# danini/pose-graph-initialization

Measured on AMD Instinct MI355X. Metric: pose-graph edges/sec (essential+decompose), higher is better.
Workload: dtype f32 scoring / f64 solver; 1 GPU; configs[1]: 10000 pairs x 2000 corrs batched essential RANSAC + decompose per GPU; pairs_per_gpu=10000, corrs_per_pair=2000, mode=adaptive (confidence 0.99, cap 1000, rounds of 32), parallelism=pairs sharded over 1 GPU(s), exchange=none (single GPU)

## Files before the change

pose-graph-initialization_amd/csrc/pgi_kernels.hip:

```cpp
#include "pgi_device.hpp"
#include "pgi_internal.hpp"

#include <algorithm>
#include <condition_variable>
#include <mutex>
#include <new>
#include <string>
#include <thread>
#include <vector>
#include <cstdio>
#include <cstdlib>
#include <cstring>

namespace pgi {

constexpr int kMaxNW = 4;
constexpr uint32_t kNw1Pairs = 98304, kNw2Pairs = 12288;
constexpr int QCAP = 40;
constexpr double QMAGIC = 393216.0;

struct GcCtx {
    uint32_t* prev;
    uint32_t* msg;
    uint8_t* lab;
    uint32_t* last;
    const float* e_lds;
    uint32_t lambda64;
    uint32_t built;
};

template <int NW>
struct WgShared {
    float bestE[9];
    int best_score;
    uint32_t best_ninl;
    float candE[NW][9];
    int cand_score[NW];
    uint32_t cand_ninl[NW];
    uint32_t cand_hyp[NW];
    uint32_t wave_cnt[NW];
    uint32_t votes[4];
    uint32_t q_count[NW];
    uint32_t q_hyp[NW][QCAP];
    uint32_t pass_ctr;
    uint32_t nbar;
    uint32_t mask_cnt;
    int lo_score;
    uint32_t lo_ninl, lo_ni, lo_runs;
    float loE[9];
    double Rt[21];
    GcCtx gc;
};

struct K1Args {
    const float* x1;
    const float* y1;
    const float* x2;
    const float* y2;
    const uint64_t* off;
    const double* thr;
    const double* guess;
    const uint8_t* has_guess;
    pgi_edge* edges;
    uint8_t* masks;
    uint32_t n_pairs;
    uint32_t pts_cap;
    uint64_t pair_id_base;
    uint64_t seed;
    pgi_params prm;
    unsigned long long* prof;
    const uint32_t* pair_list;
    const uint32_t* pair_count;
    uint32_t* pair_head;
    const float* src_x1;
    const float* src_y1;
    const float* src_x2;
    const float* src_y2;
    uint32_t* gc_prev;
    uint32_t* gc_msg;
    uint32_t gc_lds_off;
};

template <int LDS_PTS>
struct Rows {
    const float4* lds;
    const float* x1;
    const float* y1;
    const float* x2;
    const float* y2;
    uint32_t n;
    uint32_t lds_n;
    PGI_DEV float4 get(uint32_t i) const {
        if constexpr (LDS_PTS == 1) {
            return lds[i];
        } else if constexpr (LDS_PTS == 2) {
            if (i < lds_n) return lds[i];
            const float nanv = __builtin_nanf("");
            if (i < n) return make_float4(x1[i], y1[i], x2[i], y2[i]);
            return make_float4(nanv, nanv, nanv, nanv);
        } else {
            const float nanv = __builtin_nanf("");
            if (i < n) return make_float4(x1[i], y1[i], x2[i], y2[i]);
            return make_float4(nanv, nanv, nanv, nanv);
// ... 187 lines not shown
        base -= 64u;
        const uint32_t i = base + (uint32_t)lane;
        const bool valid = i < n;
        const uint32_t w = valid ? gc_load(g.msg + i) : 0u;
        const uint32_t pv = valid ? gc_load(g.prev + i) : kGcNone;
        const uint32_t k = gc_word_k(w) & 31u;
        const int d = gc_word_delta(w);
        succ_of[lane] = 64u;
        wave_sync();
        if (valid && pv != kGcNone && pv >= base) succ_of[pv - base] = (uint32_t)lane;
        wave_sync();
        const uint32_t succ = succ_of[lane];
        wave_sync();
        uint32_t lab = (w >> 6) & 1u;
        if (succ == 64u && !((w >> 5) & 1u)) lab = d < 0 ? 1u : 0u;
        bool done = !valid || succ == 64u;
        const int sl = succ == 64u ? 0 : (int)succ;
        for (;;) {
            const uint64_t dm = __ballot(done);
            if (dm == ~0ull) break;
            const uint32_t ls = (uint32_t)__shfl((int)lab, sl), ks = (uint32_t)__shfl((int)k, sl);
            if (!done && ((dm >> sl) & 1ull)) {
                lab = gc_prev_label(ls, ks, d, k, lam);
                done = true;
            }
        }
        if (valid && pv != kGcNone && pv < base) {
            const uint32_t wp = gc_load(g.msg + pv);
            gc_store(g.msg + pv, wp | 32u | (gc_prev_label(lab, k, gc_word_delta(wp), gc_word_k(wp) & 31u, lam) << 6));
        }
        if (valid) g.lab[i] = (uint8_t)lab;
        cnt += (uint32_t)__popcll(__ballot(valid && lab));
        asm volatile("s_waitcnt vmcnt(0)" ::: "memory");
    }
    wave_sync();
    return cnt;
}

template <int LDS_PTS>
__device__ __noinline__ uint32_t gc_label_rows(const float4* lds, const float* x1, const float* y1, const float* x2, const float* y2, uint32_t n,
                                               uint32_t lds_n, uint32_t npad, float thr2, GcCtx* gp, int lane) {
    Rows<LDS_PTS> rows;
    rows.lds = lds;
    rows.x1 = x1; rows.y1 = y1; rows.x2 = x2; rows.y2 = y2;
    rows.n = n;
    rows.lds_n = lds_n;
    return gc_label_wave<LDS_PTS>(&rows, n, npad, thr2, gp, lane);
}

template <int LDS_PTS>
PGI_DEV uint32_t normal_matrix_wave(const Rows<LDS_PTS>& rows, uint32_t npad, const float E[9], float tau2,
                                    double* loA, double* tri, int lane, const uint8_t* lab = nullptr) {
    uint32_t cnt = 0;
#pragma unroll
    for (int blk = 0; blk < 3; ++blk) {
        constexpr int kLo[3] = {0, 17, 35}, kRow0[3] = {0, 2, 5}, kRow1[3] = {2, 5, 9}, kCnt[3] = {17, 18, 10};
        double S[18];
#pragma unroll
        for (int i = 0; i < 18; ++i) S[i] = 0.0;
        for (uint32_t base = 0; base < npad; base += 64) {
            const float4 p = rows.get(base + lane);
            float r2, den;
            sampson_terms(E, p.x, p.y, p.z, p.w, r2, den);
            const bool in = lab ? (base + (uint32_t)lane < rows.n && lab[base + lane] != 0) : (r2 < tau2 * den);
            if (blk == 0) cnt += __popcll(__ballot(in));
            if (in) {
                const double x1 = p.x, y1 = p.y, x2 = p.z, y2 = p.w;
                double a[9];
                a[0] = x2 * x1; a[1] = x2 * y1; a[2] = x2;
                a[3] = y2 * x1; a[4] = y2 * y1; a[5] = y2;
                a[6] = x1;      a[7] = y1;      a[8] = 1.0;
                constexpr int kTri[9] = {0, 9, 17, 24, 30, 35, 39, 42, 44};
#pragma unroll
                for (int ii = kRow0[blk]; ii < kRow1[blk]; ++ii)
#pragma unroll
                    for (int jj = ii; jj < 9; ++jj) {
                        const int k = kTri[ii] + (jj - ii) - kLo[blk];
                        double t = a[ii] * a[jj];
                        t = (t + QMAGIC) - QMAGIC;
                        S[k] = S[k] + t;
                    }
            }
        }
#pragma unroll
        for (int i = 0; i < kCnt[blk]; ++i) {
            const double v = wave_sum_exact(S[i]);
            if (lane == 0) tri[kLo[blk] + i] = v;
        }
    }
    wave_sync();
    if (lane < 45) {
        int i = 0, rem = lane;
        while (rem >= 9 - i) {
            rem -= 9 - i;
            ++i;
        }
        const int j = i + rem;
        const double v = tri[lane];
        loA[9 * i + j] = v;
        loA[9 * j + i] = v;
    }
    wave_sync();
    return cnt;
}

template <int LDS_PTS, int NW>
PGI_DEV uint32_t normal_matrix_wg(const Rows<LDS_PTS>& rows, uint32_t npad, const float E[9], float tau2,
                                  double* loA, double* partial, WgShared<NW>* sh, int tid) {
    constexpr int NT = NW * 64;
    const int lane = tid & 63, w = tid >> 6;
    uint32_t cnt = 0;
#pragma unroll
    for (int blk = 0; blk < 3; ++blk) {
        constexpr int kLo[3] = {0, 17, 35}, kRow0[3] = {0, 2, 5}, kRow1[3] = {2, 5, 9}, kCnt[3] = {17, 18, 10};
        double S[18];
#pragma unroll
        for (int i = 0; i < 18; ++i) S[i] = 0.0;
        for (uint32_t base = 0; base < npad; base += NT) {
            const uint32_t i = base + tid;
            const float nanv = __builtin_nanf("");
            const float4 p = (i < npad) ? rows.get(i) : make_float4(nanv, nanv, nanv, nanv);
            float r2, den;
            sampson_terms(E, p.x, p.y, p.z, p.w, r2, den);
            const bool in = r2 < tau2 * den;
            if (blk == 0) cnt += __popcll(__ballot(in));
            if (in) {
                const double x1 = p.x, y1 = p.y, x2 = p.z, y2 = p.w;
                double a[9];
                a[0] = x2 * x1; a[1] = x2 * y1; a[2] = x2;
                a[3] = y2 * x1; a[4] = y2 * y1; a[5] = y2;
                a[6] = x1;      a[7] = y1;      a[8] = 1.0;
                constexpr int kTri[9] = {0, 9, 17, 24, 30, 35, 39, 42, 44};
#pragma unroll
                for (int ii = kRow0[blk]; ii < kRow1[blk]; ++ii)
#pragma unroll
                    for (int jj = ii; jj < 9; ++jj) {
                        const int k = kTri[ii] + (jj - ii) - kLo[blk];
                        double t = a[ii] * a[jj];
                        t = (t + QMAGIC) - QMAGIC;
                        S[k] = S[k] + t;
                    }
            }
        }
#pragma unroll
        for (int i = 0; i < kCnt[blk]; ++i) {
            const double v = wave_sum_exact(S[i]);
            if (lane == 0) partial[45 * w + kLo[blk] + i] = v;
        }
    }
    if (lane == 0) sh->wave_cnt[w] = cnt;
    __syncthreads();
    if (tid < 45) {
        double v = partial[tid];
#pragma unroll
        for (int ww = 1; ww < NW; ++ww) v = v + partial[45 * ww + tid];
        int i = 0, rem = tid;
        while (rem >= 9 - i) {
            rem -= 9 - i;
            ++i;
        }
        const int j = i + rem;
        loA[9 * i + j] = v;
        loA[9 * j + i] = v;
    }
    uint32_t total = 0;
#pragma unroll
    for (int ww = 0; ww < NW; ++ww) total += sh->wave_cnt[ww];
    __syncthreads();
    return total;
}

PGI_DEV void jacobi9_wave(double* A, double* V, double* basis0, int lane) {
    for (int i = lane; i < 81; i += 64) V[i] = (i % 10 == 0) ? 1.0 : 0.0;
    wave_sync();
    const int m = lane / 9, l = lane - 9 * m;
    const bool act = lane < 36;
    int pr = act ? m + 1 : 1, qr = act ? 8 - m : 8;
    for (int sw = 0; sw < kJacobiSweeps; ++sw)
        for (int r = 0; r < 9; ++r) {
            const int p = min(pr, qr), q = max(pr, qr);
            pr = pr == 8 ? 0 : pr + 1;
            qr = qr == 8 ? 0 : qr + 1;
            double c = 1.0, s = 0.0;
            if (act) {
                const double apq = A[9 * p + q];
                if (apq != 0.0) {
                    const double al = A[10 * q] - A[10 * p], be = 2.0 * apq;
                    const double h = sqrt(fma(al, al, be * be));
                    const double d = fabs(al) + h;
                    const double r = sqrt(fma(d, d, be * be));
                    const double inv = 1.0 / r;
                    c = d * inv;
                    s = (al >= 0.0 ? be : -be) * inv;
                }
            }
            wave_sync();
            if (act) {
                const double ap = A[9 * l + p], aq = A[9 * l + q];
                A[9 * l + p] = fma(c, ap, -(s * aq));
                A[9 * l + q] = fma(s, ap, c * aq);
                const double vp = V[9 * l + p], vq = V[9 * l + q];
                V[9 * l + p] = fma(c, vp, -(s * vq));
                V[9 * l + q] = fma(s, vp, c * vq);
            }
            wave_sync();
            if (act) {
                const double ap = A[9 * p + l], aq = A[9 * q + l];
                A[9 * p + l] = fma(c, ap, -(s * aq));
                A[9 * q + l] = fma(s, ap, c * aq);
            }
            wave_sync();
        }
    double d[9];
#pragma unroll
    for (int i = 0; i < 9; ++i) d[i] = A[10 * i];
    uint32_t taken = 0;
// ... 90 lines not shown
    double* wscr = wscr_all + w * W_DOUBLES;
    float* queue = reinterpret_cast<float*>(wscr + W_REGA);

    Rows<LDS_PTS> rows;
    rows.lds = pts;
    rows.x1 = a.x1 + o; rows.y1 = a.y1 + o; rows.x2 = a.x2 + o; rows.y2 = a.y2 + o;
    rows.n = n;
    rows.lds_n = LDS_PTS != 0 ? min(npad, a.pts_cap) : 0u;

    pgi_edge* edge = a.edges + pair;
    uint8_t* mask = a.masks + o;
    Prof prof;
    prof.start();

    if (LDS_PTS == 1 && npad > a.pts_cap) {
        for (uint32_t i = tid; i < n; i += NT) mask[i] = 0;
        if (tid == 0) {
            edge_clear(edge);
            edge->status = PGI_EDGE_TOO_MANY_ROWS;
        }
        return;
    }
    {
        const bool direct = a.src_x1 != nullptr;
        const float* sx1 = direct ? a.src_x1 + o : rows.x1;
        const float* sy1 = direct ? a.src_y1 + o : rows.y1;
        const float* sx2 = direct ? a.src_x2 + o : rows.x2;
        const float* sy2 = direct ? a.src_y2 + o : rows.y2;
        if constexpr (LDS_PTS != 0) {
            const float nanv = __builtin_nanf("");
            for (uint32_t i = tid; i < rows.lds_n; i += NT)
                pts[i] = (i < n) ? make_float4(sx1[i], sy1[i], sx2[i], sy2[i]) : make_float4(nanv, nanv, nanv, nanv);
        }
        if constexpr (LDS_PTS != 1) {
            if (direct) {
                float* mx1 = const_cast<float*>(rows.x1);
                float* my1 = const_cast<float*>(rows.y1);
                float* mx2 = const_cast<float*>(rows.x2);
                float* my2 = const_cast<float*>(rows.y2);
                for (uint32_t i = rows.lds_n + tid; i < n; i += NT) {
                    mx1[i] = sx1[i];
                    my1[i] = sy1[i];
                    mx2[i] = sx2[i];
                    my2[i] = sy2[i];
                }
            }
        }
    }
    if (tid == 0) {
        sh->best_score = -1;
        sh->best_ninl = 0;
        sh->votes[0] = sh->votes[1] = sh->votes[2] = sh->votes[3] = 0;
        sh->mask_cnt = 0;
        sh->pass_ctr = 0;
        sh->nbar = 0;
        sh->lo_runs = 0;
        if (a.gc_prev) {
            sh->gc.prev = a.gc_prev + o;
            sh->gc.msg = a.gc_msg + o;
            sh->gc.lab = mask;
            sh->gc.last = reinterpret_cast<uint32_t*>(smem + a.gc_lds_off);
            sh->gc.e_lds = sh->bestE;
            sh->gc.lambda64 = min(a.prm.lo_graph_cut, 255u);
            sh->gc.built = 0;
        }
    }
    __syncthreads();
    prof.mark<0>();

    const double thr = a.thr[pair];
    const float thr2 = (float)(thr * thr);
    const pgi_params prm = a.prm;

    if (n < 5) {
        for (uint32_t i = tid; i < n; i += NT) mask[i] = 0;
        if (tid == 0) {
            edge_clear(edge);
            edge->status = PGI_EDGE_FEW_POINTS;
        }
        return;
    }

    uint32_t out_iters = 0, out_lo = 0, out_used_guess = 0, out_score = 0;
    float mask_tau2 = thr2;
    bool success = false, have_model = false;
    uint32_t guess_ninl = 0;

    bool guided_done = false;
    auto local_optimise = [&]() {
        if constexpr (!GUESS) return;
        int ni_first = -1;
        GcCtx* const gc = a.gc_prev ? &sh->gc : nullptr;
        if constexpr (NW > 1) {
            if (prm.lo_iters && !gc) {
                float bE0[9];
#pragma unroll
                for (int c = 0; c < 9; ++c) bE0[c] = sh->bestE[c];
                int td = tid;
                asm volatile("" : "+v"(td));
                ni_first = (int)normal_matrix_wg<LDS_PTS, NW>(rows, npad, bE0, thr2, wscr_all + W_REGA + G_REGA_SZ, wscr_all + W_DOUBLES, sh, td);
            }
        }
        if (w == 0) {
            for (uint32_t it = 0; it < prm.lo_iters; ++it) {
                float bE[9];
#pragma unroll
                for (int c = 0; c < 9; ++c) bE[c] = sh->bestE[c];
                const int cur_best = __builtin_amdgcn_readfirstlane(sh->best_score);
// ... 14 lines not shown
                if (ln < 9) sh->bestE[ln] = reinterpret_cast<const float*>(wscr_all + W_REGA)[9 * r_idx + ln];
                wave_sync();
            }
        }
    };
    if (GUESS && a.has_guess[pair] && prm.guess_mode == 1u) {
        const double* G = a.guess + 12 * (size_t)pair;
        const double R[9] = {G[0], G[1], G[2], G[3], G[4], G[5], G[6], G[7], G[8]};
        const uint64_t rng_g = mix64(a.seed ^ mix64(a.pair_id_base + pair));
        int ln = lane;
        asm volatile("" : "+v"(ln));
        constexpr int kPerWave = 32 / NW;
        const bool mine = ln < kPerWave;
        const uint32_t h = (uint32_t)(w * kPerWave + (mine ? ln : 0));
        const uint32_t i0 = draw_index(rng_g, 0x40000000u + h, 0u, n);
        uint32_t i1 = i0;
        for (uint32_t k = 1; k < 64u && i1 == i0; ++k) i1 = draw_index(rng_g, 0x40000000u + h, k, n);
        double nv[2][3];
#pragma unroll
        for (int q = 0; q < 2; ++q) {
            const float4 p = rows.get(q == 0 ? i0 : i1);
            const double X1[3] = {(double)p.x, (double)p.y, 1.0}, X2[3] = {(double)p.z, (double)p.w, 1.0};
            double av[3];
#pragma unroll
            for (int i = 0; i < 3; ++i) av[i] = fma(R[3 * i], X1[0], fma(R[3 * i + 1], X1[1], R[3 * i + 2]));
            cross3(X2, av, nv[q]);
        }
        double t[3];
        cross3(nv[0], nv[1], t);
        const double t2 = fma(t[0], t[0], fma(t[1], t[1], t[2] * t[2]));
        const double tx[9] = {0, -t[2], t[1], t[2], 0, -t[0], -t[1], t[0], 0};
        double Eg[9], n2 = 0.0;
#pragma unroll
        for (int i = 0; i < 3; ++i)
#pragma unroll
            for (int j = 0; j < 3; ++j) {
                double sacc = 0;
#pragma unroll
                for (int k = 0; k < 3; ++k) sacc += tx[3 * i + k] * R[3 * k + j];
                Eg[3 * i + j] = sacc;
            }
#pragma unroll
        for (int m = 0; m < 9; ++m) n2 = fma(Eg[m], Eg[m], n2);
        const double inv = 1.0 / sqrt(n2);
        float E32[9];
#pragma unroll
        for (int m = 0; m < 9; ++m) E32[m] = (float)(Eg[m] * inv);
        const bool valid = mine && (t2 > 1e-30) && (n2 > 0.0);
        const int cnt = enqueue_models(valid, E32, h, queue, sh->q_hyp[w], ln);
        wave_sync();
        int gb_score = -1, gb_idx = -1;
        uint32_t gb_ninl = 0, gb_hyp = 0;
        score_queue<LDS_PTS>(rows, n, npad, queue, sh->q_hyp[w], 0, cnt, thr2, ln, -1, 0u, gb_score, gb_ninl, gb_hyp, gb_idx);
        if (gb_idx >= 0 && ln < 9) sh->candE[w][ln] = queue[9 * gb_idx + ln];
        if (lane == 0) {
            sh->cand_score[w] = gb_score;
            sh->cand_ninl[w] = gb_ninl;
            sh->cand_hyp[w] = gb_hyp;
        }
        __syncthreads();
        int rb = -1, rbw = -1;
        uint32_t rbh = 0;
#pragma unroll
        for (int ww = 0; ww < NW; ++ww) {
            const int cs = sh->cand_score[ww];
            const uint32_t ch = sh->cand_hyp[ww];
            if (cs > rb || (cs == rb && cs >= 0 && ch < rbh)) {
                rb = cs;
                rbw = ww;
                rbh = ch;
            }
        }
        __syncthreads();
        if (rb >= 0) {
            if (tid == 0) {
                sh->best_score = rb;
                sh->best_ninl = sh->cand_ninl[rbw];
#pragma unroll
                for (int c = 0; c < 9; ++c) sh->bestE[c] = sh->candE[rbw][c];
            }
            __syncthreads();
            local_optimise();
            __syncthreads();
            if (sh->best_ninl >= prm.min_inliers) {
                guided_done = true;
                have_model = true;
                out_used_guess = 1;
                out_iters = 32;
                out_lo = sh->lo_runs;
                out_score = (uint32_t)sh->best_score;
            }
        }
        if (!guided_done) {
            __syncthreads();
            if (tid == 0) {
                sh->best_score = -1;
                sh->best_ninl = 0;
                sh->lo_runs = 0;
            }
            __syncthreads();
        }
    }

    if (GUESS && a.has_guess[pair] && prm.guess_mode != 1u) {
        const double* G = a.guess + 12 * (size_t)pair;
        const double R[9] = {G[0], G[1], G[2], G[3], G[4], G[5], G[6], G[7], G[8]};
        const double t[3] = {G[9], G[10], G[11]};
        const double tx[9] = {0, -t[2], t[1], t[2], 0, -t[0], -t[1], t[0], 0};
        double Eg[9], n2 = 0.0;
#pragma unroll
        for (int i = 0; i < 3; ++i)
#pragma unroll
            for (int j = 0; j < 3; ++j) {
                double s = 0;
#pragma unroll
                for (int k = 0; k < 3; ++k) s += tx[3 * i + k] * R[3 * k + j];
                Eg[3 * i + j] = s;
            }
#pragma unroll
        for (int m = 0; m < 9; ++m) n2 = fma(Eg[m], Eg[m], n2);
        const double inv = 1.0 / sqrt(n2);
        float Ef[9];
#pragma unroll
        for (int m = 0; m < 9; ++m) Ef[m] = (float)(Eg[m] * inv);
        const double trunc = 1.5 * thr;
        const float tau2 = prm.guess_quirk ? (float)trunc : (float)(trunc * trunc);
        if (w == 0) {
            __builtin_amdgcn_s_setprio(3);
            int rs0, ri0;
            uint32_t rn0;
            const uint32_t ni0 = refit_wave0<LDS_PTS>(rows, n, npad, Ef, tau2, thr2, wscr_all, sh->q_hyp[0], lane, -1, 0u, rs0, rn0, ri0, prof);
            if (lane == 0) {
                sh->lo_ni = ni0;
                sh->lo_score = rs0;
                sh->lo_ninl = rn0;
            }
            if (ri0 >= 0 && lane < 9) sh->loE[lane] = reinterpret_cast<const float*>(wscr_all + W_REGA)[9 * ri0 + lane];
            __builtin_amdgcn_s_setprio(0);
        }
        __syncthreads();
        const uint32_t ni = sh->lo_ni;
        const int r_score = sh->lo_score;
        if (ni >= 5 && r_score >= 0 && ni >= prm.min_inliers) {
            success = true;
            have_model = true;
            out_used_guess = 1;
            out_lo = 1;
            out_score = (uint32_t)r_score;
            guess_ninl = ni;
            mask_tau2 = tau2;
            if (tid == 0) {
#pragma unroll
                for (int c = 0; c < 9; ++c) sh->bestE[c] = Ef[c];
            }
            __syncthreads();
        }
    }

    if (!success && !guided_done) {
        const uint64_t rng_base = mix64(a.seed ^ mix64(a.pair_id_base + pair));
        const uint32_t rs = prm.round_size ? prm.round_size : 32u;
        const uint32_t budget = prm.fixed_budget ? prm.fixed_budget : prm.max_iters;
        uint32_t hyps = 0;
        const uint32_t n_pass = (rs + 3u) / 4u;
        int wb_score = -1;
        uint32_t wb_ninl = 0, wb_hyp = 0;
        auto do_pass = [&](uint32_t pass, uint32_t base_hyp, int floor_score, uint32_t n_bar) {
            int ln = lane;
            asm volatile("" : "+v"(ln));
            const int g = ln >> 4, s = ln & 15;
            const uint32_t local = pass * 4 + g;
            const bool active = local < rs;
            const uint32_t hyp = base_hyp + (active ? local : 0u);
            const GroupScratch gs = group_scratch(wscr, g);
            uint32_t idx[5];
            sample5_group(rng_base, hyp, prm.sampler ? progressive_rows(hyp, n, prm.max_iters) : n, s, g * 16, ln,
                          reinterpret_cast<uint32_t*>(gs.rega), idx);
            uint32_t my = idx[0];
#pragma unroll
            for (int k = 1; k < 5; ++k)
                if (s == k) my = idx[k];
            const float4 mine = rows.get(my);
            prof.mark<1>();
            nullspace5_group(mine, s, g * 16, gs);
            prof.mark<2>();
            float E32[9];
            if constexpr (LDS_PTS != 1) {
                if (s < 5) smp_stash[(w * 4 + g) * 5 + s] = mine;
                wave_sync();
            }
            const bool valid = backend_group<false, 3, true>(
                gs, s, g * 16,
                [&](int i) {
                    if constexpr (LDS_PTS == 1) return rows.get(idx[i]);
                    else return smp_stash[(w * 4 + g) * 5 + i];
                },
                E32, nullptr, prof);
            wave_sync();
            const int cnt = enqueue_models(valid && active, E32, hyp, queue, sh->q_hyp[w], ln);
            wave_sync();
            prof.mark<9>();
            int bidx = -1;
            score_queue<LDS_PTS>(rows, n, npad, queue, sh->q_hyp[w], 0, cnt, thr2, ln, floor_score, n_bar, wb_score,
                                 wb_ninl, wb_hyp, bidx);
            if (bidx >= 0 && ln < 9) sh->candE[w][ln] = queue[9 * bidx + ln];
            wave_sync();
            prof.mark<10>();
        };
        auto pull_pass = [&]() -> uint32_t {
            uint32_t pass = 0;
            if (lane == 0) pass = atomicAdd(&sh->pass_ctr, 1u);
            return (uint32_t)__builtin_amdgcn_readfirstlane((int)pass);
        };
        int floor_score = -1;
        uint32_t n_bar = 0;
        bool deferred = false;
        auto terminated = [&](uint32_t at_hyps) {
            if (prm.fixed_budget || sh->best_score < 0 || sh->best_ninl < 5) return false;
            uint32_t nn = n;
            double conf = prm.confidence;
            asm volatile("" : "+s"(nn), "+s"(conf));
            const double rho = (double)sh->best_ninl / (double)nn;
            const double r5 = ((rho * rho) * (rho * rho)) * rho;
            const double q = 1.0 - r5;
            return pow_uint(q, at_hyps) <= 1.0 - conf;
        };
        while (hyps < budget) {
            for (;;) {
                const uint32_t pass = pull_pass();
                if (pass >= n_pass) break;
                do_pass(pass, hyps, floor_score, n_bar);
            }
            if (lane == 0) {
                sh->cand_score[w] = wb_score;
                sh->cand_ninl[w] = wb_ninl;
                sh->cand_hyp[w] = wb_hyp;
            }
            wb_score = -1;
            __syncthreads();
            prof.mark<22>();
            if (deferred) {
                deferred = false;
                if (terminated(hyps)) break;
            }
            hyps += rs;
            int rb = -1, rbw = -1;
            uint32_t rbh = 0;
#pragma unroll
            for (int ww = 0; ww < NW; ++ww) {
                const int cs = sh->cand_score[ww];
                const uint32_t ch = sh->cand_hyp[ww];
                if (cs > rb || (cs == rb && cs >= 0 && ch < rbh)) {
                    rb = cs;
                    rbw = ww;
                    rbh = ch;
                }
            }
            const bool improve = (rb >= 0) && (rb > sh->best_score);
            __syncthreads();
            if (tid == 0) {
                sh->pass_ctr = 0;
                if (improve) {
                    sh->best_score = rb;
                    sh->best_ninl = sh->cand_ninl[rbw];
                    sh->nbar = sh->cand_ninl[rbw];
#pragma unroll
                    for (int c = 0; c < 9; ++c) sh->bestE[c] = sh->candE[rbw][c];
                } else {
                    sh->nbar = sh->best_score >= 0 ? sh->best_ninl : 0u;
                }
            }
            __syncthreads();
            floor_score = __builtin_amdgcn_readfirstlane(sh->best_score);
            n_bar = (uint32_t)__builtin_amdgcn_readfirstlane((int)sh->nbar);
            if (improve) {
                int ni_first = -1;
                GcCtx* const gc = a.gc_prev ? &sh->gc : nullptr;
                if (NW > 1 && prm.lo_iters && !gc) {
                    float bE0[9];
#pragma unroll
                    for (int c = 0; c < 9; ++c) bE0[c] = sh->bestE[c];
                    const int td = (w << 6) + fresh_lane_id();
                    ni_first = (int)normal_matrix_wg<LDS_PTS, NW>(rows, npad, bE0, thr2, wscr_all + W_REGA + G_REGA_SZ,
                                                              wscr_all + W_DOUBLES, sh, td);
                }
                if (w == 0) {
                    __builtin_amdgcn_s_setprio(3);
                    for (uint32_t it = 0; it < prm.lo_iters; ++it) {
                        float bE[9];
#pragma unroll
                        for (int c = 0; c < 9; ++c) bE[c] = sh->bestE[c];
                        const int cur_best = __builtin_amdgcn_readfirstlane(sh->best_score);
                        const uint32_t cur_ninl = (uint32_t)__builtin_amdgcn_readfirstlane((int)sh->best_ninl);
                        int r_score, r_idx;
                        uint32_t r_ninl;
                        int ln = lane;
                        asm volatile("" : "+v"(ln));
                        const uint32_t ni = refit_wave0<LDS_PTS>(rows, n, npad, bE, thr2, thr2, wscr_all, sh->q_hyp[0], ln, cur_best,
                                                                       cur_ninl, r_score, r_ninl, r_idx, prof,
                                                                       it == 0 ? ni_first : -1, prm.lo_linear_pct, gc);
                        if (ni < 5) break;
                        if (lane == 0) sh->lo_runs += 1;
                        if (!(r_score > cur_best)) break;
                        if (lane == 0) {
                            sh->best_score = r_score;
                            sh->best_ninl = r_ninl;
                        }
                        if (ln < 9) sh->bestE[ln] = reinterpret_cast<const float*>(wscr_all + W_REGA)[9 * r_idx + ln];
                        wave_sync();
                    }
                    __builtin_amdgcn_s_setprio(0);
                }
                if constexpr (NW == 1) {
                    if (terminated(hyps)) break;
                } else {
                    deferred = true;
                }
            } else if (terminated(hyps)) {
                break;
            }
        }
        __syncthreads();
        out_lo = sh->lo_runs;
        out_iters = hyps;
        have_model = sh->best_score >= 0;
        if (have_model) out_score = (uint32_t)sh->best_score;
    }

    prof.mark<23>();
    const int ew = w, etid = (ew << 6) + fresh_lane_id(), elane = etid & 63;
    if (!have_model) {
        for (uint32_t i = etid; i < n; i += NT) mask[i] = 0;
        if (etid == 0) {
            edge_clear(edge);
            edge->status = PGI_EDGE_FEW_INLIERS;
            edge->iters = out_iters;
            edge->lo_runs = out_lo;
        }
        return;
    }
    const float* finalE = success ? sh->loE : sh->bestE;
    float maskE[9];
#pragma unroll
    for (int c = 0; c < 9; ++c) maskE[c] = sh->bestE[c];
    uint32_t mc = 0;
    if (ew == 0) decompose_wave(finalE, sh->Rt, elane);
    if (NW == 1 || ew != 0) {
        constexpr uint32_t kMaskLanes = NW == 1 ? 64u : (uint32_t)(NT - 64);
        for (uint32_t base = 0; base < npad; base += kMaskLanes) {
            const uint32_t i = base + (uint32_t)(NW == 1 ? etid : etid - 64);
            const float nanv = __builtin_nanf("");
            const float4 p = (i < npad) ? rows.get(i) : make_float4(nanv, nanv, nanv, nanv);
            float r2, den;
            sampson_terms(maskE, p.x, p.y, p.z, p.w, r2, den);
            const bool in = r2 < mask_tau2 * den;
            if (i < n) mask[i] = in ? 1 : 0;
            mc += __popcll(__ballot(in));
        }
        if (elane == 0) atomicAdd(&sh->mask_cnt, mc);
    }
    __syncthreads();
    double R1[9], R2[9], tt[3];
#pragma unroll
    for (int c = 0; c < 9; ++c) {
        R1[c] = sh->Rt[c];
        R2[c] = sh->Rt[9 + c];
    }
    tt[0] = sh->Rt[18]; tt[1] = sh->Rt[19]; tt[2] = sh->Rt[20];
    uint32_t v0 = 0, v1 = 0, v2 = 0, v3 = 0;
    for (uint32_t base = 0; base < npad; base += NT) {
        const uint32_t i = base + etid;
        const float nanv = __builtin_nanf("");
        const float4 p = (i < npad) ? rows.get(i) : make_float4(nanv, nanv, nanv, nanv);
        float r2, den;
        sampson_terms(maskE, p.x, p.y, p.z, p.w, r2, den);
        const bool in = r2 < mask_tau2 * den;
        const bool voter = (i < n) && (prm.vote_all_rows || in);
        uint32_t b1 = 0, b2 = 0;
        if (voter) {
            const double X1[3] = {p.x, p.y, 1.0}, X2[3] = {p.z, p.w, 1.0};
            double x2t[3];
            cross3(X2, tt, x2t);
            b1 = cheirality_bits(R1, tt, X1, X2, x2t);
            b2 = cheirality_bits(R2, tt, X1, X2, x2t);
        }
        v0 += __popcll(__ballot(b1 & 1u));
        v1 += __popcll(__ballot(b1 & 2u));
        v2 += __popcll(__ballot(b2 & 1u));
        v3 += __popcll(__ballot(b2 & 2u));
    }
    if (elane == 0) {
        atomicAdd(&sh->votes[0], v0);
        atomicAdd(&sh->votes[1], v1);
        atomicAdd(&sh->votes[2], v2);
        atomicAdd(&sh->votes[3], v3);
    }
    __syncthreads();
    if (etid == 0) {
        edge_clear(edge);
        const uint32_t n_inl = success ? guess_ninl : sh->mask_cnt;
#pragma unroll
        for (int c = 0; c < 9; ++c) edge->E[c] = (double)finalE[c];
        edge->n_inl = n_inl;
        edge->score = out_score;
        edge->iters = out_iters;
        edge->lo_runs = out_lo;
        edge->used_guess = out_used_guess;
        if (n_inl < prm.min_inliers) {
            edge->status = PGI_EDGE_FEW_INLIERS;
        } else {
            const uint32_t vt0 = sh->votes[0], vt1 = sh->votes[1], vt2 = sh->votes[2], vt3 = sh->votes[3];
            uint32_t best = 0, bv = vt0;
            if (vt1 > bv) { bv = vt1; best = 1; }
            if (vt2 > bv) { bv = vt2; best = 2; }
            if (vt3 > bv) { bv = vt3; best = 3; }
            const bool second = (best >> 1) != 0;
            bool bad = false;
#pragma unroll
            for (int c = 0; c < 9; ++c) {
                const double rv = second ? R2[c] : R1[c];
                edge->R[c] = rv;
                bad |= !(rv == rv);
            }
#pragma unroll
            for (int c = 0; c < 3; ++c) {
                edge->t[c] = (best & 1u) ? -tt[c] : tt[c];
                bad |= !(tt[c] == tt[c]);
            }
            edge->votes = bv;
            edge->cand = best;
// ... 1344 lines not shown
```

pose-graph-initialization_amd/csrc/pgi_device.hpp:

```cpp
#pragma once
#include <hip/hip_runtime.h>
#include <stdint.h>

#define PGI_DEV __device__ __forceinline__
#define PGI_PHASE __device__ __noinline__

namespace pgi {

constexpr int kGrid = 256;
constexpr int kNewton = 10;
constexpr int kJacobiSweeps = 6;
constexpr int kSvdSweeps = 4;
constexpr int kMaxModels = 10;

constexpr int kProfSlots = 32;
#ifdef PGI_PROFILE
struct Prof {
    unsigned long long t, acc[kProfSlots];
    PGI_DEV void start() {
        for (int i = 0; i < kProfSlots; ++i) acc[i] = 0;
        t = __builtin_amdgcn_s_memtime();
    }
    template <int I>
    PGI_DEV void mark() {
        const unsigned long long n = __builtin_amdgcn_s_memtime();
        acc[I] += n - t;
        t = n;
    }
    PGI_DEV void flush(unsigned long long* out, int lane) {
        if (out && lane == 0)
            for (int i = 0; i < kProfSlots; ++i) atomicAdd(out + i, acc[i]);
    }
};
#else
struct Prof {
    PGI_DEV void start() {}
    template <int I>
    PGI_DEV void mark() {}
    PGI_DEV void flush(unsigned long long*, int) {}
};
#endif

PGI_DEV void wave_sync() {
    __builtin_amdgcn_fence(__ATOMIC_RELEASE, "wavefront");
    __builtin_amdgcn_wave_barrier();
    __builtin_amdgcn_fence(__ATOMIC_ACQUIRE, "wavefront");
}

template <int CTRL>
PGI_DEV int dpp_i(int v) {
    return __builtin_amdgcn_update_dpp(0, v, CTRL, 0xF, 0xF, true);
}
template <int CTRL>
PGI_DEV double dpp_d(double v) {
    const int lo = __double2loint(v), hi = __double2hiint(v);
// ... 761 lines not shown
```

pose-graph-initialization_amd/pyposegraphbuilder/_lib.py:

```python
import ctypes as C
import os

import numpy as np

_PKG = os.path.dirname(os.path.abspath(__file__))
LIB_PATH = os.path.join(os.path.dirname(_PKG), "libpgi.so")
DBG_DOUBLES = 358


class Params(C.Structure):
    _fields_ = [("confidence", C.c_double), ("max_iters", C.c_uint32), ("round_size", C.c_uint32),
                ("lo_iters", C.c_uint32), ("min_inliers", C.c_uint32), ("fixed_budget", C.c_uint32),
                ("guess_quirk", C.c_uint32), ("vote_all_rows", C.c_uint32), ("guess_mode", C.c_uint32),
                ("lo_linear_pct", C.c_uint32), ("sampler", C.c_uint32), ("lo_graph_cut", C.c_uint32)]


class Edge(C.Structure):
    _fields_ = [("E", C.c_double * 9), ("R", C.c_double * 9), ("t", C.c_double * 3),
                ("status", C.c_int32), ("n_inl", C.c_uint32), ("score", C.c_uint32),
                ("iters", C.c_uint32), ("votes", C.c_uint32), ("cand", C.c_uint32),
                ("used_guess", C.c_uint32), ("lo_runs", C.c_uint32)]


class Batch(C.Structure):
# ... 182 lines not shown
    lib.pgi_five_point_batch.argtypes = [C.c_void_p, C.c_void_p, C.c_uint32, C.c_void_p, C.c_void_p, C.c_void_p]
    lib.pgi_rotation_average.argtypes = [C.c_void_p, C.c_void_p, C.c_uint32, C.c_uint32,
                                         C.POINTER(RotAvgParams), C.c_void_p, C.c_void_p]
    lib.pgi_default_rotavg_params.argtypes = [C.POINTER(RotAvgParams)]
    lib.pgi_default_transavg_params.argtypes = [C.POINTER(TransAvgParams)]
    lib.pgi_translation_average.argtypes = [C.c_void_p, C.c_void_p, C.c_uint32, C.c_uint32,
                                            C.POINTER(TransAvgParams), C.c_void_p, C.c_void_p]
    lib.pgi_translation_average_edges.argtypes = [C.c_void_p, C.c_void_p, C.c_void_p, C.c_void_p, C.c_void_p, C.c_uint32, C.c_uint32,
                                                  C.c_void_p, C.POINTER(TransAvgParams), C.c_void_p, C.c_void_p, C.c_void_p]
    lib.pgi_default_triangulate_params.restype = None
    lib.pgi_default_triangulate_params.argtypes = [C.POINTER(TriangulateParams)]
    view_args = [C.POINTER(KeypointView), C.c_void_p, C.c_void_p, C.c_void_p, C.c_uint32, C.POINTER(TriangulateParams)]
    lib.pgi_triangulate_tracks.argtypes = [C.c_void_p, C.c_void_p, C.c_void_p, C.c_uint32] + view_args + [C.c_void_p] * 6
    lib.pgi_tracklets_triangulate.argtypes = [C.c_void_p] + view_args + [C.c_void_p] * 6
    lib.pgi_default_bundle_params.restype = None
    lib.pgi_default_bundle_params.argtypes = [C.POINTER(BundleParams)]
    ba_args = [C.POINTER(KeypointView), C.c_void_p, C.c_void_p, C.c_void_p, C.c_void_p, C.c_uint32, C.POINTER(BundleParams),
               C.c_void_p, C.c_void_p, C.c_void_p, C.POINTER(BundleReport)]
    lib.pgi_bundle_adjust.argtypes = [C.c_void_p, C.c_void_p, C.c_void_p, C.c_uint32] + ba_args
    lib.pgi_tracklets_bundle_adjust.argtypes = [C.c_void_p] + ba_args
    baf_args = ba_args[:-1] + [C.c_void_p, C.c_void_p, C.c_uint32, C.POINTER(BundleReport), C.POINTER(C.c_uint32)]
    lib.pgi_bundle_adjust_focal.argtypes = [C.c_void_p, C.c_void_p, C.c_void_p, C.c_uint32] + baf_args
    lib.pgi_tracklets_bundle_adjust_focal.argtypes = [C.c_void_p] + baf_args
    lib.pgi_default_cycle_params.restype = None
    lib.pgi_default_cycle_params.argtypes = [C.POINTER(CycleParams)]
    lib.pgi_cycle_filter.argtypes = [C.c_void_p, C.c_void_p, C.c_uint32, C.c_uint32, C.POINTER(CycleParams), C.c_void_p, C.c_void_p,
                                     C.c_void_p, C.POINTER(CycleSummary)]
    lib.pgi_cycle_filter_edges.argtypes = [C.c_void_p, C.c_void_p, C.c_void_p, C.c_void_p, C.c_uint32, C.c_uint32, C.POINTER(CycleParams),
                                           C.c_void_p, C.c_void_p, C.c_void_p, C.POINTER(CycleSummary), C.c_void_p]
    _lib = lib
    return lib


def last_error():
    return load().pgi_last_error().decode()


def check(rc):
    if rc < 0:
        raise PgiError("pgi error %d: %s" % (rc, last_error()))
    return rc


def default_params(**kw):
    p = Params()
    load().pgi_default_params(C.byref(p))
    for k, v in kw.items():
        if not hasattr(p, k):
            raise TypeError("unknown parameter %r" % k)
        setattr(p, k, v)
    return p


def kernel_source_sha256(files=("csrc/pgi_kernels.hip", "csrc/pgi_device.hpp")):
    import hashlib
    h = hashlib.sha256()
    root = os.path.dirname(_PKG)
    for f in files:
        with open(os.path.join(root, f), "rb") as fh:
            h.update(fh.read())
    return h.hexdigest()
```

Baseline: 1.701 million edges/s.

## Double-buffer round candidates to drop a barrier and cache inlier bits

Candidate and pass-counter state is double-buffered by round parity. Each wave now reads the published best score and picks the round winner itself, which removes one of the two workgroup barriers per adaptive round. The normal-matrix builders keep the first block's inlier test as a per-lane bitmask and reuse it in later blocks instead of recomputing Sampson errors. The decompose vote pass reads inlier ballots stored in wave scratch during the mask pass, and the Rt buffer moves from shared state into scratch. This adds subtle cross-wave ordering assumptions and shrinks the shared struct, at the cost of more code complexity and possible race risk.

```diff
diff --git a/pose-graph-initialization_amd/csrc/pgi_kernels.hip b/pose-graph-initialization_amd/csrc/pgi_kernels.hip
--- a/pose-graph-initialization_amd/csrc/pgi_kernels.hip
+++ b/pose-graph-initialization_amd/csrc/pgi_kernels.hip
@@ -34,21 +34,21 @@
     float bestE[9];
     int best_score;
     uint32_t best_ninl;
-    float candE[NW][9];
-    int cand_score[NW];
-    uint32_t cand_ninl[NW];
-    uint32_t cand_hyp[NW];
+    float candE[2][NW][9];
+    int cand_score[2][NW];
+    uint32_t cand_ninl[2][NW];
+    uint32_t cand_hyp[2][NW];
+    int pub_score[2];
+    uint32_t pub_ninl[2];
     uint32_t wave_cnt[NW];
     uint32_t votes[4];
     uint32_t q_count[NW];
     uint32_t q_hyp[NW][QCAP];
-    uint32_t pass_ctr;
-    uint32_t nbar;
+    uint32_t pass_ctr[2];
     uint32_t mask_cnt;
     int lo_score;
     uint32_t lo_ninl, lo_ni, lo_runs;
     float loE[9];
-    double Rt[21];
     GcCtx gc;
 };
 
@@ -342,6 +342,7 @@
 PGI_DEV uint32_t normal_matrix_wave(const Rows<LDS_PTS>& rows, uint32_t npad, const float E[9], float tau2,
                                     double* loA, double* tri, int lane, const uint8_t* lab = nullptr) {
     uint32_t cnt = 0;
+    uint64_t inm = 0;
 #pragma unroll
     for (int blk = 0; blk < 3; ++blk) {
         constexpr int kLo[3] = {0, 17, 35}, kRow0[3] = {0, 2, 5}, kRow1[3] = {2, 5, 9}, kCnt[3] = {17, 18, 10};
@@ -350,9 +351,18 @@
         for (int i = 0; i < 18; ++i) S[i] = 0.0;
         for (uint32_t base = 0; base < npad; base += 64) {
             const float4 p = rows.get(base + lane);
-            float r2, den;
-            sampson_terms(E, p.x, p.y, p.z, p.w, r2, den);
-            const bool in = lab ? (base + (uint32_t)lane < rows.n && lab[base + lane] != 0) : (r2 < tau2 * den);
+            const uint32_t step = base >> 6;
+            bool in;
+            if (lab) {
+                in = base + (uint32_t)lane < rows.n && lab[base + lane] != 0;
+            } else if (blk == 0 || step >= 64u) {
+                float r2, den;
+                sampson_terms(E, p.x, p.y, p.z, p.w, r2, den);
+                in = r2 < tau2 * den;
+                if (blk == 0 && step < 64u) inm |= (uint64_t)(in ? 1u : 0u) << step;
+            } else {
+                in = ((inm >> step) & 1u) != 0;
+            }
             if (blk == 0) cnt += __popcll(__ballot(in));
             if (in) {
                 const double x1 = p.x, y1 = p.y, x2 = p.z, y2 = p.w;
@@ -400,19 +410,27 @@
     constexpr int NT = NW * 64;
     const int lane = tid & 63, w = tid >> 6;
     uint32_t cnt = 0;
+    uint64_t inm = 0;
 #pragma unroll
     for (int blk = 0; blk < 3; ++blk) {
         constexpr int kLo[3] = {0, 17, 35}, kRow0[3] = {0, 2, 5}, kRow1[3] = {2, 5, 9}, kCnt[3] = {17, 18, 10};
         double S[18];
 #pragma unroll
         for (int i = 0; i < 18; ++i) S[i] = 0.0;
-        for (uint32_t base = 0; base < npad; base += NT) {
+        uint32_t step = 0;
+        for (uint32_t base = 0; base < npad; base += NT, ++step) {
             const uint32_t i = base + tid;
             const float nanv = __builtin_nanf("");
             const float4 p = (i < npad) ? rows.get(i) : make_float4(nanv, nanv, nanv, nanv);
-            float r2, den;
-            sampson_terms(E, p.x, p.y, p.z, p.w, r2, den);
-            const bool in = r2 < tau2 * den;
+            bool in;
+            if (blk == 0 || step >= 64u) {
+                float r2, den;
+                sampson_terms(E, p.x, p.y, p.z, p.w, r2, den);
+                in = r2 < tau2 * den;
+                if (blk == 0 && step < 64u) inm |= (uint64_t)(in ? 1u : 0u) << step;
+            } else {
+                in = ((inm >> step) & 1u) != 0;
+            }
             if (blk == 0) cnt += __popcll(__ballot(in));
             if (in) {
                 const double x1 = p.x, y1 = p.y, x2 = p.z, y2 = p.w;
@@ -648,8 +666,7 @@
         sh->best_ninl = 0;
         sh->votes[0] = sh->votes[1] = sh->votes[2] = sh->votes[3] = 0;
         sh->mask_cnt = 0;
-        sh->pass_ctr = 0;
-        sh->nbar = 0;
+        sh->pass_ctr[0] = sh->pass_ctr[1] = 0;
         sh->lo_runs = 0;
         if (a.gc_prev) {
             sh->gc.prev = a.gc_prev + o;
@@ -770,19 +787,19 @@
         int gb_score = -1, gb_idx = -1;
         uint32_t gb_ninl = 0, gb_hyp = 0;
         score_queue<LDS_PTS>(rows, n, npad, queue, sh->q_hyp[w], 0, cnt, thr2, ln, -1, 0u, gb_score, gb_ninl, gb_hyp, gb_idx);
-        if (gb_idx >= 0 && ln < 9) sh->candE[w][ln] = queue[9 * gb_idx + ln];
+        if (gb_idx >= 0 && ln < 9) sh->candE[0][w][ln] = queue[9 * gb_idx + ln];
         if (lane == 0) {
-            sh->cand_score[w] = gb_score;
-            sh->cand_ninl[w] = gb_ninl;
-            sh->cand_hyp[w] = gb_hyp;
+            sh->cand_score[0][w] = gb_score;
+            sh->cand_ninl[0][w] = gb_ninl;
+            sh->cand_hyp[0][w] = gb_hyp;
         }
         __syncthreads();
         int rb = -1, rbw = -1;
         uint32_t rbh = 0;
 #pragma unroll
         for (int ww = 0; ww < NW; ++ww) {
-            const int cs = sh->cand_score[ww];
-            const uint32_t ch = sh->cand_hyp[ww];
+            const int cs = sh->cand_score[0][ww];
+            const uint32_t ch = sh->cand_hyp[0][ww];
             if (cs > rb || (cs == rb && cs >= 0 && ch < rbh)) {
                 rb = cs;
                 rbw = ww;
@@ -793,9 +810,9 @@
         if (rb >= 0) {
             if (tid == 0) {
                 sh->best_score = rb;
-                sh->best_ninl = sh->cand_ninl[rbw];
-#pragma unroll
-                for (int c = 0; c < 9; ++c) sh->bestE[c] = sh->candE[rbw][c];
+                sh->best_ninl = sh->cand_ninl[0][rbw];
+#pragma unroll
+                for (int c = 0; c < 9; ++c) sh->bestE[c] = sh->candE[0][rbw][c];
             }
             __syncthreads();
             local_optimise();
@@ -883,6 +900,7 @@
         const uint32_t n_pass = (rs + 3u) / 4u;
         int wb_score = -1;
         uint32_t wb_ninl = 0, wb_hyp = 0;
+        uint32_t par = 0;
         auto do_pass = [&](uint32_t pass, uint32_t base_hyp, int floor_score, uint32_t n_bar) {
             int ln = lane;
             asm volatile("" : "+v"(ln));
@@ -921,24 +939,24 @@
             int bidx = -1;
             score_queue<LDS_PTS>(rows, n, npad, queue, sh->q_hyp[w], 0, cnt, thr2, ln, floor_score, n_bar, wb_score,
                                  wb_ninl, wb_hyp, bidx);
-            if (bidx >= 0 && ln < 9) sh->candE[w][ln] = queue[9 * bidx + ln];
+            if (bidx >= 0 && ln < 9) sh->candE[par][w][ln] = queue[9 * bidx + ln];
             wave_sync();
             prof.mark<10>();
         };
         auto pull_pass = [&]() -> uint32_t {
             uint32_t pass = 0;
-            if (lane == 0) pass = atomicAdd(&sh->pass_ctr, 1u);
+            if (lane == 0) pass = atomicAdd(&sh->pass_ctr[par], 1u);
             return (uint32_t)__builtin_amdgcn_readfirstlane((int)pass);
         };
         int floor_score = -1;
         uint32_t n_bar = 0;
         bool deferred = false;
-        auto terminated = [&](uint32_t at_hyps) {
-            if (prm.fixed_budget || sh->best_score < 0 || sh->best_ninl < 5) return false;
+        auto terminated = [&](int cur_score, uint32_t cur_ninl, uint32_t at_hyps) {
+            if (prm.fixed_budget || cur_score < 0 || cur_ninl < 5) return false;
             uint32_t nn = n;
             double conf = prm.confidence;
             asm volatile("" : "+s"(nn), "+s"(conf));
-            const double rho = (double)sh->best_ninl / (double)nn;
+            const double rho = (double)cur_ninl / (double)nn;
             const double r5 = ((rho * rho) * (rho * rho)) * rho;
             const double q = 1.0 - r5;
             return pow_uint(q, at_hyps) <= 1.0 - conf;
@@ -950,54 +968,64 @@
                 do_pass(pass, hyps, floor_score, n_bar);
             }
             if (lane == 0) {
-                sh->cand_score[w] = wb_score;
-                sh->cand_ninl[w] = wb_ninl;
-                sh->cand_hyp[w] = wb_hyp;
+                sh->cand_score[par][w] = wb_score;
+                sh->cand_ninl[par][w] = wb_ninl;
+                sh->cand_hyp[par][w] = wb_hyp;
+                if (w == 0) {
+                    sh->pub_score[par] = sh->best_score;
+                    sh->pub_ninl[par] = sh->best_ninl;
+                }
             }
             wb_score = -1;
             __syncthreads();
             prof.mark<22>();
+            int best_score = __builtin_amdgcn_readfirstlane(sh->pub_score[par]);
+            uint32_t best_ninl = (uint32_t)__builtin_amdgcn_readfirstlane((int)sh->pub_ninl[par]);
             if (deferred) {
                 deferred = false;
-                if (terminated(hyps)) break;
+                if (terminated(best_score, best_ninl, hyps)) break;
             }
             hyps += rs;
             int rb = -1, rbw = -1;
             uint32_t rbh = 0;
 #pragma unroll
             for (int ww = 0; ww < NW; ++ww) {
-                const int cs = sh->cand_score[ww];
-                const uint32_t ch = sh->cand_hyp[ww];
+                const int cs = sh->cand_score[par][ww];
+                const uint32_t ch = sh->cand_hyp[par][ww];
                 if (cs > rb || (cs == rb && cs >= 0 && ch < rbh)) {
                     rb = cs;
                     rbw = ww;
                     rbh = ch;
                 }
             }
-            const bool improve = (rb >= 0) && (rb > sh->best_score);
-            __syncthreads();
-            if (tid == 0) {
-                sh->pass_ctr = 0;
-                if (improve) {
-                    sh->best_score = rb;
-                    sh->best_ninl = sh->cand_ninl[rbw];
-                    sh->nbar = sh->cand_ninl[rbw];
-#pragma unroll
-                    for (int c = 0; c < 9; ++c) sh->bestE[c] = sh->candE[rbw][c];
-                } else {
-                    sh->nbar = sh->best_score >= 0 ? sh->best_ninl : 0u;
+            rb = __builtin_amdgcn_readfirstlane(rb);
+            rbw = __builtin_amdgcn_readfirstlane(rbw);
+            const bool improve = (rb >= 0) && (rb > best_score);
+            if (improve) {
+                best_score = rb;
+                best_ninl = (uint32_t)__builtin_amdgcn_readfirstlane((int)sh->cand_ninl[par][rbw]);
+            }
+            floor_score = best_score;
+            n_bar = best_score >= 0 ? best_ninl : 0u;
+            if (w == 0) {
+                const int fl = fresh_lane_id();
+                if (fl == 0) {
+                    sh->pass_ctr[par] = 0;
+                    if (improve) {
+                        sh->best_score = best_score;
+                        sh->best_ninl = best_ninl;
+                    }
                 }
-            }
-            __syncthreads();
-            floor_score = __builtin_amdgcn_readfirstlane(sh->best_score);
-            n_bar = (uint32_t)__builtin_amdgcn_readfirstlane((int)sh->nbar);
+                if (improve && fl < 9) sh->bestE[fl] = sh->candE[par][rbw][fl];
+                wave_sync();
+            }
             if (improve) {
                 int ni_first = -1;
                 GcCtx* const gc = a.gc_prev ? &sh->gc : nullptr;
                 if (NW > 1 && prm.lo_iters && !gc) {
                     float bE0[9];
 #pragma unroll
-                    for (int c = 0; c < 9; ++c) bE0[c] = sh->bestE[c];
+                    for (int c = 0; c < 9; ++c) bE0[c] = sh->candE[par][rbw][c];
                     const int td = (w << 6) + fresh_lane_id();
                     ni_first = (int)normal_matrix_wg<LDS_PTS, NW>(rows, npad, bE0, thr2, wscr_all + W_REGA + G_REGA_SZ,
                                                               wscr_all + W_DOUBLES, sh, td);
@@ -1030,13 +1058,16 @@
                     __builtin_amdgcn_s_setprio(0);
                 }
                 if constexpr (NW == 1) {
-                    if (terminated(hyps)) break;
+                    if (terminated(__builtin_amdgcn_readfirstlane(sh->best_score),
+                                   (uint32_t)__builtin_amdgcn_readfirstlane((int)sh->best_ninl), hyps))
+                        break;
                 } else {
                     deferred = true;
                 }
-            } else if (terminated(hyps)) {
+            } else if (terminated(best_score, best_ninl, hyps)) {
                 break;
             }
+            par ^= 1u;
         }
         __syncthreads();
         out_lo = sh->lo_runs;
@@ -1061,8 +1092,11 @@
     float maskE[9];
 #pragma unroll
     for (int c = 0; c < 9; ++c) maskE[c] = sh->bestE[c];
+    double* const Rt = wscr_all;
+    uint32_t* const inl_bal = reinterpret_cast<uint32_t*>(wscr_all + 22);
+    constexpr uint32_t kBalSteps = (uint32_t)(NW * W_DOUBLES - 22);
     uint32_t mc = 0;
-    if (ew == 0) decompose_wave(finalE, sh->Rt, elane);
+    if (ew == 0) decompose_wave(finalE, Rt, elane);
     if (NW == 1 || ew != 0) {
         constexpr uint32_t kMaskLanes = NW == 1 ? 64u : (uint32_t)(NT - 64);
         for (uint32_t base = 0; base < npad; base += kMaskLanes) {
@@ -1073,7 +1107,10 @@
             sampson_terms(maskE, p.x, p.y, p.z, p.w, r2, den);
             const bool in = r2 < mask_tau2 * den;
             if (i < n) mask[i] = in ? 1 : 0;
-            mc += __popcll(__ballot(in));
+            const uint64_t bal = __ballot(in);
+            mc += __popcll(bal);
+            const uint32_t st = (base >> 6) + (uint32_t)(NW == 1 ? 0 : ew - 1);
+            if (st < kBalSteps && elane < 2 && i < npad) inl_bal[2 * st + elane] = (uint32_t)(bal >> (32 * elane));
         }
         if (elane == 0) atomicAdd(&sh->mask_cnt, mc);
     }
@@ -1081,19 +1118,28 @@
     double R1[9], R2[9], tt[3];
 #pragma unroll
     for (int c = 0; c < 9; ++c) {
-        R1[c] = sh->Rt[c];
-        R2[c] = sh->Rt[9 + c];
-    }
-    tt[0] = sh->Rt[18]; tt[1] = sh->Rt[19]; tt[2] = sh->Rt[20];
+        R1[c] = Rt[c];
+        R2[c] = Rt[9 + c];
+    }
+    tt[0] = Rt[18]; tt[1] = Rt[19]; tt[2] = Rt[20];
     uint32_t v0 = 0, v1 = 0, v2 = 0, v3 = 0;
     for (uint32_t base = 0; base < npad; base += NT) {
         const uint32_t i = base + etid;
         const float nanv = __builtin_nanf("");
         const float4 p = (i < npad) ? rows.get(i) : make_float4(nanv, nanv, nanv, nanv);
-        float r2, den;
-        sampson_terms(maskE, p.x, p.y, p.z, p.w, r2, den);
-        const bool in = r2 < mask_tau2 * den;
-        const bool voter = (i < n) && (prm.vote_all_rows || in);
+        bool voter = i < n;
+        if (!prm.vote_all_rows) {
+            const uint32_t st = (base >> 6) + (uint32_t)ew;
+            bool in = false;
+            if (st >= kBalSteps) {
+                float r2, den;
+                sampson_terms(maskE, p.x, p.y, p.z, p.w, r2, den);
+                in = r2 < mask_tau2 * den;
+            } else if (voter) {
+                in = ((inl_bal[2 * st + (uint32_t)(elane >> 5)] >> (elane & 31)) & 1u) != 0;
+            }
+            voter = voter && in;
+        }
         uint32_t b1 = 0, b2 = 0;
         if (voter) {
             const double X1[3] = {p.x, p.y, 1.0}, X2[3] = {p.z, p.w, 1.0};
```

After: 1.710 million edges/s, median of 5. Within noise of the previous version (+0.5%).

## Exploit Kronecker symmetry to accumulate 36 normal-matrix monomials instead of 45

Applied to the files above, without the earlier changes.

The 8-point design row a = x2 ⊗ x1 makes many entries of the 9x9 normal matrix duplicates: a[i]*a[j] equals a[i2]*a[j2] when the indices swap factors. The accumulation now sums only 36 unique monomials in two passes of 18 instead of 45 entries in three passes, and a scatter step writes each value to up to four matrix positions. This cuts the number of passes over the points, the fp64 multiply/quantize/add work per inlier and the wave reductions. It relies on the quantized products being bitwise identical for twin entries, which holds because the products are exactly equal.

```diff
diff --git a/pose-graph-initialization_amd/csrc/pgi_device.hpp b/pose-graph-initialization_amd/csrc/pgi_device.hpp
--- a/pose-graph-initialization_amd/csrc/pgi_device.hpp
+++ b/pose-graph-initialization_amd/csrc/pgi_device.hpp
@@ -1,6 +1,8 @@
 #pragma once
 #include <hip/hip_runtime.h>
 #include <stdint.h>
+
+#include "pgi_normal_monomials.hpp"
 
 #define PGI_DEV __device__ __forceinline__
 #define PGI_PHASE __device__ __noinline__
diff --git a/pose-graph-initialization_amd/csrc/pgi_kernels.hip b/pose-graph-initialization_amd/csrc/pgi_kernels.hip
--- a/pose-graph-initialization_amd/csrc/pgi_kernels.hip
+++ b/pose-graph-initialization_amd/csrc/pgi_kernels.hip
@@ -17,7 +17,6 @@
 constexpr int kMaxNW = 4;
 constexpr uint32_t kNw1Pairs = 98304, kNw2Pairs = 12288;
 constexpr int QCAP = 40;
-constexpr double QMAGIC = 393216.0;
 
 struct GcCtx {
     uint32_t* prev;
@@ -343,11 +342,10 @@
                                     double* loA, double* tri, int lane, const uint8_t* lab = nullptr) {
     uint32_t cnt = 0;
 #pragma unroll
-    for (int blk = 0; blk < 3; ++blk) {
-        constexpr int kLo[3] = {0, 17, 35}, kRow0[3] = {0, 2, 5}, kRow1[3] = {2, 5, 9}, kCnt[3] = {17, 18, 10};
-        double S[18];
-#pragma unroll
-        for (int i = 0; i < 18; ++i) S[i] = 0.0;
+    for (int blk = 0; blk < 2; ++blk) {
+        double S[kNormalPass];
+#pragma unroll
+        for (int i = 0; i < kNormalPass; ++i) S[i] = 0.0;
         for (uint32_t base = 0; base < npad; base += 64) {
             const float4 p = rows.get(base + lane);
             float r2, den;
@@ -355,41 +353,19 @@
             const bool in = lab ? (base + (uint32_t)lane < rows.n && lab[base + lane] != 0) : (r2 < tau2 * den);
             if (blk == 0) cnt += __popcll(__ballot(in));
             if (in) {
-                const double x1 = p.x, y1 = p.y, x2 = p.z, y2 = p.w;
                 double a[9];
-                a[0] = x2 * x1; a[1] = x2 * y1; a[2] = x2;
-                a[3] = y2 * x1; a[4] = y2 * y1; a[5] = y2;
-                a[6] = x1;      a[7] = y1;      a[8] = 1.0;
-                constexpr int kTri[9] = {0, 9, 17, 24, 30, 35, 39, 42, 44};
-#pragma unroll
-                for (int ii = kRow0[blk]; ii < kRow1[blk]; ++ii)
-#pragma unroll
-                    for (int jj = ii; jj < 9; ++jj) {
-                        const int k = kTri[ii] + (jj - ii) - kLo[blk];
-                        double t = a[ii] * a[jj];
-                        t = (t + QMAGIC) - QMAGIC;
-                        S[k] = S[k] + t;
-                    }
-            }
-        }
-#pragma unroll
-        for (int i = 0; i < kCnt[blk]; ++i) {
+                normal_design_row(p.x, p.y, p.z, p.w, a);
+                if (blk == 0) normal_accumulate<0>(a, S); else normal_accumulate<1>(a, S);
+            }
+        }
+#pragma unroll
+        for (int i = 0; i < kNormalPass; ++i) {
             const double v = wave_sum_exact(S[i]);
-            if (lane == 0) tri[kLo[blk] + i] = v;
+            if (lane == 0) tri[kNormalPass * blk + i] = v;
         }
     }
     wave_sync();
-    if (lane < 45) {
-        int i = 0, rem = lane;
-        while (rem >= 9 - i) {
-            rem -= 9 - i;
-            ++i;
-        }
-        const int j = i + rem;
-        const double v = tri[lane];
-        loA[9 * i + j] = v;
-        loA[9 * j + i] = v;
-    }
+    if (lane < kNormalMonomials) normal_scatter(lane, tri[lane], loA);
     wave_sync();
     return cnt;
 }
@@ -401,11 +377,10 @@
     const int lane = tid & 63, w = tid >> 6;
     uint32_t cnt = 0;
 #pragma unroll
-    for (int blk = 0; blk < 3; ++blk) {
-        constexpr int kLo[3] = {0, 17, 35}, kRow0[3] = {0, 2, 5}, kRow1[3] = {2, 5, 9}, kCnt[3] = {17, 18, 10};
-        double S[18];
-#pragma unroll
-        for (int i = 0; i < 18; ++i) S[i] = 0.0;
+    for (int blk = 0; blk < 2; ++blk) {
+        double S[kNormalPass];
+#pragma unroll
+        for (int i = 0; i < kNormalPass; ++i) S[i] = 0.0;
         for (uint32_t base = 0; base < npad; base += NT) {
             const uint32_t i = base + tid;
             const float nanv = __builtin_nanf("");
@@ -415,43 +390,24 @@
             const bool in = r2 < tau2 * den;
             if (blk == 0) cnt += __popcll(__ballot(in));
             if (in) {
-                const double x1 = p.x, y1 = p.y, x2 = p.z, y2 = p.w;
                 double a[9];
-                a[0] = x2 * x1; a[1] = x2 * y1; a[2] = x2;
-                a[3] = y2 * x1; a[4] = y2 * y1; a[5] = y2;
-                a[6] = x1;      a[7] = y1;      a[8] = 1.0;
-                constexpr int kTri[9] = {0, 9, 17, 24, 30, 35, 39, 42, 44};
-#pragma unroll
-                for (int ii = kRow0[blk]; ii < kRow1[blk]; ++ii)
-#pragma unroll
-                    for (int jj = ii; jj < 9; ++jj) {
-                        const int k = kTri[ii] + (jj - ii) - kLo[blk];
-                        double t = a[ii] * a[jj];
-                        t = (t + QMAGIC) - QMAGIC;
-                        S[k] = S[k] + t;
-                    }
-            }
-        }
-#pragma unroll
-        for (int i = 0; i < kCnt[blk]; ++i) {
+                normal_design_row(p.x, p.y, p.z, p.w, a);
+                if (blk == 0) normal_accumulate<0>(a, S); else normal_accumulate<1>(a, S);
+            }
+        }
+#pragma unroll
+        for (int i = 0; i < kNormalPass; ++i) {
             const double v = wave_sum_exact(S[i]);
-            if (lane == 0) partial[45 * w + kLo[blk] + i] = v;
+            if (lane == 0) partial[kNormalMonomials * w + kNormalPass * blk + i] = v;
         }
     }
     if (lane == 0) sh->wave_cnt[w] = cnt;
     __syncthreads();
-    if (tid < 45) {
+    if (tid < kNormalMonomials) {
         double v = partial[tid];
 #pragma unroll
-        for (int ww = 1; ww < NW; ++ww) v = v + partial[45 * ww + tid];
-        int i = 0, rem = tid;
-        while (rem >= 9 - i) {
-            rem -= 9 - i;
-            ++i;
-        }
-        const int j = i + rem;
-        loA[9 * i + j] = v;
-        loA[9 * j + i] = v;
+        for (int ww = 1; ww < NW; ++ww) v = v + partial[kNormalMonomials * ww + tid];
+        normal_scatter(tid, v, loA);
     }
     uint32_t total = 0;
 #pragma unroll
diff --git a/pose-graph-initialization_amd/csrc/pgi_normal_monomials.hpp b/pose-graph-initialization_amd/csrc/pgi_normal_monomials.hpp
--- /dev/null
+++ b/pose-graph-initialization_amd/csrc/pgi_normal_monomials.hpp
@@ -0,0 +1,68 @@
+#pragma once
+#include <stdint.h>
+
+#if defined(__HIPCC__)
+#define PGI_HD __host__ __device__ __forceinline__
+#define PGI_UNROLL _Pragma("unroll")
+#else
+#define PGI_HD inline
+#define PGI_UNROLL
+#endif
+
+namespace pgi {
+
+constexpr double QMAGIC = 393216.0;
+
+constexpr int kNormalMonomials = 36;
+constexpr int kNormalPass = 18;
+
+constexpr uint32_t kSymLo = 0u | (0u << 2) | (0u << 4) | (1u << 6) | (1u << 8) | (2u << 10);
+constexpr uint32_t kSymHi = 0u | (1u << 2) | (2u << 4) | (1u << 6) | (2u << 8) | (2u << 10);
+
+struct NormalMonomial {
+    int i, j, i2, j2;
+};
+PGI_HD constexpr NormalMonomial normal_monomial(int k) {
+    const int P = k / 6, Q = k - 6 * P;
+    const int p = (int)((kSymLo >> (2 * P)) & 3u), r = (int)((kSymHi >> (2 * P)) & 3u);
+    const int q = (int)((kSymLo >> (2 * Q)) & 3u), s = (int)((kSymHi >> (2 * Q)) & 3u);
+    const bool twin = p != r && q != s;
+    return NormalMonomial{3 * p + q, 3 * r + s, twin ? 3 * p + s : 3 * p + q, twin ? 3 * r + q : 3 * r + s};
+}
+struct NormalMonomialTab {
+    NormalMonomial m[kNormalMonomials];
+};
+constexpr NormalMonomialTab make_normal_monomials() {
+    NormalMonomialTab t{};
+    for (int k = 0; k < kNormalMonomials; ++k) t.m[k] = normal_monomial(k);
+    return t;
+}
+constexpr NormalMonomialTab kNormalTab = make_normal_monomials();
+
+PGI_HD void normal_design_row(float fx1, float fy1, float fx2, float fy2, double a[9]) {
+    const double x1 = fx1, y1 = fy1, x2 = fx2, y2 = fy2;
+    a[0] = x2 * x1; a[1] = x2 * y1; a[2] = x2;
+    a[3] = y2 * x1; a[4] = y2 * y1; a[5] = y2;
+    a[6] = x1;      a[7] = y1;      a[8] = 1.0;
+}
+
+template <int PASS>
+PGI_HD void normal_accumulate(const double a[9], double S[kNormalPass]) {
+    PGI_UNROLL
+    for (int k = 0; k < kNormalPass; ++k) {
+        constexpr NormalMonomialTab T = make_normal_monomials();
+        double t = a[T.m[kNormalPass * PASS + k].i] * a[T.m[kNormalPass * PASS + k].j];
+        t = (t + QMAGIC) - QMAGIC;
+        S[k] = S[k] + t;
+    }
+}
+
+PGI_HD void normal_scatter(int k, double v, double* A) {
+    const NormalMonomial m = normal_monomial(k);
+    A[9 * m.i + m.j] = v;
+    A[9 * m.j + m.i] = v;
+    A[9 * m.i2 + m.j2] = v;
+    A[9 * m.j2 + m.i2] = v;
+}
+
+}
diff --git a/pose-graph-initialization_amd/pyposegraphbuilder/_lib.py b/pose-graph-initialization_amd/pyposegraphbuilder/_lib.py
--- a/pose-graph-initialization_amd/pyposegraphbuilder/_lib.py
+++ b/pose-graph-initialization_amd/pyposegraphbuilder/_lib.py
@@ -258,7 +258,7 @@
     return p
 
 
-def kernel_source_sha256(files=("csrc/pgi_kernels.hip", "csrc/pgi_device.hpp")):
+def kernel_source_sha256(files=("csrc/pgi_kernels.hip", "csrc/pgi_device.hpp", "csrc/pgi_normal_monomials.hpp")):
     import hashlib
     h = hashlib.sha256()
     root = os.path.dirname(_PKG)
```

Result: faster. 1.716 million edges/s before, 1.782 million edges/s after (median of 6 runs) (+3.8%).
